# araray/sygnals

Hardware: AMD Instinct MI355X
Metric: Msamples/s STFT->MFCC (n_fft=2048, hop=512) (higher is better)
Workload: dtype f32; 1 GPU; C2: 1024 x 1 s @ 48 kHz clips per GPU, STFT n_fft=2048 hop=512 hann center -> 40-band Slaney mel -> power_to_db(ref=max, top_db=80) -> 13 MFCC (DCT-II ortho); clips_per_gpu=1024, clip_samples=48000, sr=48000, n_fft=2048, hop=512, n_mels=40, n_mfcc=13, rows_per_clip=13, parallelism=clip-sharded x1

## Files before the change

sygnals_amd/csrc/stft_mel.hip:

```cpp
#include "common.h"
#include <stdlib.h>
#include <string.h>

#define SETPRIO(n) __builtin_amdgcn_s_setprio(n)
#include "stft_dev.h"

namespace syg {
namespace {

constexpr bool X2_MEL = true;
constexpr int NFFT = 2048;
constexpr int MC = 1024;
constexpr int NBIN = 1025;
constexpr int MAXW = 16;
constexpr int P_STRIDE = 1090;
constexpr int PL2 = 132;
constexpr int SC_COMPLEX = 4 * PL2;
constexpr int TW2_STRIDE = 18;
constexpr int TW2_FLOATS = 4 * TW2_STRIDE * 2;
constexpr int TW1_FLOATS = 15 * 64 * 2;

struct MelPlan {
  int steps;
  int n_groups;
  int table_off;
};
constexpr int MTAB_INTS = 256;
constexpr int SEGTAB_WORDS = 2 * 2 * 64 * 4;
constexpr int SEGTAB4_WORDS = 2 * SEGTAB_WORDS;
constexpr int TRI4_ROW_BASE = 4;

struct ContrastPlan {
  int n_rows;
  int ascending;
  int lo[SYG_MAX_BANDS];
  int hi[SYG_MAX_BANDS];
  int k[SYG_MAX_BANDS];
};

typedef float v4f __attribute__((ext_vector_type(4)));

#include "row_features.h"

struct MfccArgs {
  const float* dct;
  const float* lifter;
  float* out;
  int n_mfcc;
  int ref_is_max;
  float ref_value, amin, top_db;
  int tp;
  int rows_per_clip;
};

__device__ __forceinline__ int x2g(int c, int cp) { return (cp & 7) * 16 + ((c + 4 * ((cp & 7) >> 1)) & 15); }

struct LaneConst {
  float2 twb[2];
  float2 cA2, cA3;
  int pkb[2];
  int pmb[2];
  int dA2, dA3;
  int kb[2];
  int g0[2], g1[2];
};

template <bool TWB = true>
__device__ __forceinline__ void init_lane_const(LaneConst& lc, int lane, const float2* __restrict__ twid) {
  constexpr float C1 = 0.92387953251128673848f, S1 = 0.38268343236508977173f, R = 0.70710678118654752440f;
#pragma unroll
  for (int j = 0; j < 2; ++j) {
    const int u = lane + 64 * j, c = u >> 3, cp = u & 7;
    int cm = 16 - c, cmp = 15 - cp;
    if (c == 0) { cm = 0; cmp = (cp == 0) ? 8 : 16 - cp; }
    lc.g0[j] = x2g(c, cp);
    lc.g1[j] = x2g(cm, cmp);
    const int kb = c + 16 * cp;
    lc.kb[j] = kb;
    lc.pkb[j] = ppos(kb);
    lc.pmb[j] = ppos(MC - kb);
    if (TWB) lc.twb[j] = twid[kb];
  }
  const bool sp = (lane == 0);
  lc.cA2 = sp ? make_float2(C1, -S1) : make_float2(0.f, -1.f);
  lc.cA3 = sp ? make_float2(S1, -C1) : make_float2(-R, -R);
  lc.dA2 = sp ? ppos(128) : 544;
  lc.dA3 = sp ? ppos(384) : 816;
}

template <int PD = 0, bool X2 = false>
__device__ __forceinline__ void wave_rfft2048(float2 (&v)[16], const LaneConst& lc, float2* __restrict__ sc,
                                             const float2* __restrict__ tw1l, const float2* __restrict__ tw2l,
                                             int lane, float2 (&xs)[2][4], float2 (&xm)[2][4], float2& x512 TARGS) {
  const int cl = lane >> 2, bp = lane & 3;
  dft16(v);
#pragma unroll
  for (int c = 1; c < 16; ++c) v[c] = cmul(v[c], tw1l[(c - 1) * 64 + lane]);
  TICK(1, v[1].x);
  float2 t[16];
  {
    const int r7 = cl & 7;
    const int rbase = r7 * 64 + bp + 8 * (cl & 8) / 2;
#pragma unroll
    for (int h = 0; h < 2; ++h) {
#pragma unroll
      for (int r = 0; r < 8; ++r) sc[r * 64 + (lane ^ (4 * r))] = v[8 * h + r];
      wave_lds_sync();
#pragma unroll
      for (int i = 0; i < 8; ++i) t[8 * h + i] = sc[rbase + 4 * (i ^ r7)];
      wave_lds_sync();
    }
#pragma unroll
    for (int i = 0; i < 8; ++i) {
      const auto sx = __builtin_amdgcn_permlane32_swap(__float_as_uint(t[i].x), __float_as_uint(t[8 + i].x), false, false);
      const auto sy = __builtin_amdgcn_permlane32_swap(__float_as_uint(t[i].y), __float_as_uint(t[8 + i].y), false, false);
      t[i] = make_float2(__uint_as_float(sx[0]), __uint_as_float(sy[0]));
      t[8 + i] = make_float2(__uint_as_float(sx[1]), __uint_as_float(sy[1]));
    }
  }
  TICK(2, t[0].x);
  SETPRIO(2 - PD > 0 ? 2 - PD : 0);
  dft16(t);
  {
    typedef __attribute__((address_space(3))) const v4f* lds_v4;
    lds_v4 t4 = (lds_v4)(tw2l + bp * TW2_STRIDE);
#pragma unroll
    for (int m = 0; m < 8; ++m) {
      const v4f tt = t4[m];
      if (m > 0) t[2 * m] = cmul(t[2 * m], make_float2(tt.x, tt.y));
      t[2 * m + 1] = cmul(t[2 * m + 1], make_float2(tt.z, tt.w));
    }
  }
  TICK(3, t[1].x);
  float2 G[2][4], H[2][4];
  {
    const int wbase = bp * PL2;
#pragma unroll
    for (int h = 0; h < 2; ++h) {
#pragma unroll
      for (int r = 0; r < 8; ++r) sc[wbase + r * 16 + ((cl + 4 * (r >> 1)) & 15)] = t[8 * h + r];
      wave_lds_sync();
#pragma unroll
      for (int j = 0; j < 2; ++j) {
        const float2* p = sc + (h == 0 ? lc.g0[j] : lc.g1[j]);
        if (h == 0) bfly4(p[0], p[PL2], p[2 * PL2], p[3 * PL2], G[j][0], G[j][1], G[j][2], G[j][3]);
        else bfly4(p[0], p[PL2], p[2 * PL2], p[3 * PL2], H[j][0], H[j][1], H[j][2], H[j][3]);
      }
      wave_lds_sync();
    }
  }
  TICK(4, G[0][0].x);
  SETPRIO(1 - PD > 0 ? 1 - PD : 0);
  x512 = X2 ? make_float2(2.f * G[0][2].x, -2.f * G[0][2].y)
            : make_float2(G[0][2].x, -G[0][2].y);
#pragma unroll
  for (int j = 0; j < 2; ++j) {
    float2 zk[4] = {G[j][0], G[j][1], G[j][2], G[j][3]};
    float2 zm[4] = {H[j][3], H[j][2], H[j][1], H[j][0]};
    if (j == 0) {
      const bool sp = (lane == 0);
      zk[2] = sp ? H[0][0] : zk[2];
      zk[3] = sp ? H[0][1] : zk[3];
      zm[0] = sp ? G[0][0] : zm[0];
      zm[1] = sp ? G[0][3] : zm[1];
      zm[2] = sp ? H[0][3] : zm[2];
      zm[3] = sp ? H[0][2] : zm[3];
    }
#pragma unroll
    for (int d = 0; d < 4; ++d) {
      const float2 E = make_float2(zk[d].x + zm[d].x, zk[d].y - zm[d].y);
      const float2 O = make_float2(zk[d].y + zm[d].y, zm[d].x - zk[d].x);
      constexpr float R = 0.70710678118654752440f;
      float2 rO;
      if (d == 0) rO = O;
      else if (d == 1) rO = make_float2(R * (O.x + O.y), R * (O.y - O.x));
      else if (j == 0) rO = cmul(O, d == 2 ? lc.cA2 : lc.cA3);
      else if (d == 2) rO = make_float2(O.y, -O.x);
      else rO = make_float2(R * (O.y - O.x), -R * (O.x + O.y));
      const float2 wO = cmul(lc.twb[j], rO);
      if (X2) {
        xs[j][d] = make_float2(E.x + wO.x, E.y + wO.y);
        xm[j][d] = make_float2(E.x - wO.x, wO.y - E.y);
      } else {
        xs[j][d] = make_float2(0.5f * (E.x + wO.x), 0.5f * (E.y + wO.y));
        xm[j][d] = make_float2(0.5f * (E.x - wO.x), -0.5f * (E.y - wO.y));
      }
    }
  }
}

template <int LOAD>
__device__ __forceinline__ void fetch_frame(float2 (&v)[16], const float* __restrict__ yb, int64_t L, int64_t s0,
                                            const float* __restrict__ stage_frame, int lane) {
  if (LOAD == 2) {
    const float2* sf = reinterpret_cast<const float2*>(stage_frame);
#pragma unroll
    for (int a = 0; a < 16; ++a) v[a] = sf[64 * a + lane];
    return;
  }
  const bool interior = (s0 >= 0) && (s0 + NFFT <= L);
  if (interior) {
#pragma unroll
    for (int a = 0; a < 16; ++a) {
      const int n = 64 * a + lane;
      if (LOAD == 1) v[a] = *reinterpret_cast<const float2*>(yb + s0 + 2 * n);
      else v[a] = make_float2(yb[s0 + 2 * n], yb[s0 + 2 * n + 1]);
    }
  } else {
#pragma unroll
    for (int a = 0; a < 16; ++a) {
      const int64_t s = s0 + 2 * (64 * a + lane);
      v[a].x = (s >= 0 && s < L) ? yb[s] : 0.f;
      v[a].y = (s + 1 >= 0 && s + 1 < L) ? yb[s + 1] : 0.f;
    }
  }
}

__device__ __forceinline__ void apply_window(float2 (&v)[16], const float2* __restrict__ winl, int lane) {
#pragma unroll
  for (int a = 0; a < 16; ++a) {
    const float2 wv = winl[64 * a + lane];
    v[a] = make_float2(v[a].x * wv.x, v[a].y * wv.y);
  }
}

template <int WAVES>
__device__ __forceinline__ void stage_tile(const float* yb, int clip_bytes, float* stage, int s_begin, int span,
                                           bool wide, int w, int lane) {
  typedef __attribute__((address_space(3))) void* lds_ptr;
  const auto rs = __builtin_amdgcn_make_buffer_rsrc(const_cast<float*>(yb), 0, clip_bytes, 0x00020000);
  if (wide) {
    const int n = (span + 255) >> 8;
    for (int c = w; c < n; c += WAVES)
      __builtin_amdgcn_raw_ptr_buffer_load_lds(rs, (lds_ptr)(stage + c * 256), 16, (s_begin + c * 256 + lane * 4) * 4,
                                               0, 0, 0);
  } else {
    const int n = (span + 63) >> 6;
    for (int c = w; c < n; c += WAVES)
      __builtin_amdgcn_raw_ptr_buffer_load_lds(rs, (lds_ptr)(stage + c * 64), 4, (s_begin + c * 64 + lane) * 4, 0, 0,
                                               0);
  }
}
__device__ __forceinline__ MfccArgs uni(const MfccArgs& a) {
  MfccArgs u;
  u.dct = uni(a.dct); u.lifter = uni(a.lifter); u.out = uni(a.out); u.n_mfcc = uni(a.n_mfcc);
  u.ref_is_max = uni(a.ref_is_max); u.ref_value = uni(a.ref_value); u.amin = uni(a.amin); u.top_db = uni(a.top_db);
  u.tp = uni(a.tp); u.rows_per_clip = uni(a.rows_per_clip);
  return u;
}

typedef __attribute__((address_space(3))) float* lds_fptr;
#include "mel_segments.h"

template <int WAVES>
__device__ __noinline__ void clip_dct(int clipmel_addr, int red_addr, int dct_addr, MfccArgs mfv, int n_mels_v, int T_v, int b_v,
                                      int w_v, int lane, int stride_v = WAVES) {
  const MfccArgs mf = uni(mfv);
  const int n_mels = uni(n_mels_v), T = uni(T_v), w = uni(w_v), stride = uni(stride_v);
  const int64_t b = uni(b_v);
  lds_fptr clipmel = (lds_fptr)(uintptr_t)(uint32_t)uni(clipmel_addr);
  lds_fptr red = (lds_fptr)(uintptr_t)(uint32_t)uni(red_addr);
  lds_fptr dctl = (lds_fptr)(uintptr_t)(uint32_t)uni(dct_addr);
  lds_fptr lifl = dctl + mf.n_mfcc * n_mels;
  float m = red[lane & (WAVES - 1)];
  m = fmaxf(m, dpp_f<DPP_QP_1032>(m));
  m = fmaxf(m, dpp_f<DPP_QP_2301>(m));
  m = fmaxf(m, dpp_f<DPP_ROW_HALF_MIRROR>(m));
  m = fmaxf(m, dpp_f<DPP_ROW_MIRROR>(m));
  constexpr float DB_PER_LOG2 = 3.01029995663981195f;
  const float ref = mf.ref_is_max ? m : fabsf(mf.ref_value);
  const float reflog = __builtin_amdgcn_logf(fmaxf(mf.amin, ref));
  const float flo = (mf.top_db >= 0.f) ? DB_PER_LOG2 * (__builtin_amdgcn_logf(fmaxf(mf.amin, m)) - reflog) - mf.top_db
                                       : -3.4e38f;
  const int ktiles = (mf.n_mfcc + 15) >> 4, ttiles = mf.tp >> 4;
  const int f = lane & 15, g = lane >> 4;
  for (int ot = w; ot < ktiles * ttiles; ot += stride) {
    const int kt = ot / ttiles, tq = ot - kt * ttiles;
    const int krow = kt * 16 + f, tcol = tq * 16 + f;
    v4f acc = {0.f, 0.f, 0.f, 0.f};
    for (int m0 = 0; m0 < n_mels; m0 += 16) {
      float a[4], bv[4];
#pragma unroll
      for (int i = 0; i < 4; ++i) {
        const int mm = m0 + 4 * i + g;
        const bool ok = mm < n_mels;
        a[i] = (krow < mf.n_mfcc && ok) ? dctl[krow * n_mels + mm] : 0.f;
        bv[i] = ok ? clipmel[mm * mf.tp + tcol] : 1.f;
      }
#pragma unroll
      for (int i = 0; i < 4; ++i) {
        const float db = fmaxf(DB_PER_LOG2 * (__builtin_amdgcn_logf(fmaxf(mf.amin, bv[i])) - reflog), flo);
        acc = __builtin_amdgcn_mfma_f32_16x16x4f32(a[i], db, acc, 0, 0, 0);
      }
    }
#pragma unroll
    for (int r = 0; r < 4; ++r) {
      const int k = kt * 16 + 4 * g + r;
      if (k < mf.n_mfcc && tcol < T) {
        float val = acc[r];
        if (mf.lifter) val *= lifl[k];
        mf.out[(b * mf.rows_per_clip + k) * (int64_t)T + tcol] = val;
      }
    }
  }
}

template <int WAVES, bool SLAB = true, int NPASS = 2>
struct Lds {
  static constexpr int TILE_T = WAVES;
  static constexpr int O_P = (NPASS == 4) ? 16 : 0;
  static constexpr int P_FLOATS = O_P + TILE_T * P_STRIDE + 16;
  static constexpr int SLAB_FLOATS = SLAB ? WAVES * 16 * TILE_T : 0;
  static constexpr int SEG_WORDS = NPASS * (SEGTAB_WORDS / 2);
  static constexpr int CPL_FLOATS = SLAB ? 3 * SYG_MAX_BANDS + MTAB_INTS : SEG_WORDS + 3 * SYG_MAX_BANDS;
  static constexpr int STAGE_FLOATS = (WAVES - 1) * 512 + NFFT;
  static constexpr int O_SLAB = P_FLOATS;
  static constexpr int O_TW2 = O_SLAB + SLAB_FLOATS;
  static constexpr int O_TW1 = O_TW2 + TW2_FLOATS;
  static constexpr int O_CPL = O_TW1 + TW1_FLOATS;
  static constexpr int O_WIN = O_CPL + CPL_FLOATS;
  static constexpr int O_STAGE = O_WIN + NFFT;
  static constexpr int TOTAL = O_STAGE + STAGE_FLOATS;
  static_assert(SC_COMPLEX * 2 <= P_STRIDE, "exchange scratch must fit inside a power row");
  static_assert(O_TW2 % 4 == 0 && O_WIN % 4 == 0 && O_STAGE % 4 == 0 && O_CPL % 4 == 0, "16-byte aligned LDS sections");
};

template <int WAVES, int LOAD, int MODE>
__global__ __launch_bounds__(WAVES * 64, 4) void stft2048_kernel(
    const float* __restrict__ y, int64_t L, int64_t ldy, int hop, int pad, int64_t T, int tiles_per_clip,
    int64_t total_tiles, int tiles_per_wg, const float2* __restrict__ win2, const float2* __restrict__ twid,
    const float* __restrict__ wpacked, MelPlan plan, int n_mels, float* __restrict__ mel_out, float binhz,
    float roll_percent, float bw_p, int smask, float* __restrict__ stats_out, ContrastPlan cplan,
    float* __restrict__ contrast_out, float2* __restrict__ cout, int dma_wide, MfccArgs mf) {
  constexpr bool TRIMEL = (MODE >= 8 && MODE <= 11);
  constexpr bool TRI = (MODE == 6 || MODE == 7 || TRIMEL);
  constexpr int NPASS = (MODE == 8 || MODE == 9) ? 4 : 2;
  constexpr int TRI_ROW_BASE = (NPASS == 4) ? TRI4_ROW_BASE : 0;
  typedef Lds<WAVES, !TRI, NPASS> LM;
  constexpr int SEG_WORDS = LM::SEG_WORDS;
  constexpr int NTHREADS = WAVES * 64;
  constexpr int TILE_T = WAVES;
  constexpr bool COMPLEX_OUT = (MODE == 2);
  constexpr bool ROWFN = (MODE == 1 || MODE == 7 || MODE == 9 || MODE == 11);
  constexpr bool CLIPM = (MODE == 3 || MODE == 6 || MODE == 7);
  constexpr bool X2 = X2_MEL && (MODE == 0 || MODE == 3 || MODE == 6 || MODE == 8 || MODE == 10);
#ifdef SYG_DEV_NO_RELC
  constexpr bool RELC = false;
#else
  constexpr bool RELC = (MODE == 7);
#endif
  constexpr float MELSC = X2 ? 0.25f : 1.f;
  extern __shared__ __attribute__((aligned(16))) float lds[];
  float* Pbuf = lds + LM::O_P;
  float* slab = lds + LM::O_SLAB;
  float2* tw2l = reinterpret_cast<float2*>(lds + LM::O_TW2);
  float2* tw1l = reinterpret_cast<float2*>(lds + LM::O_TW1);
  int* cpl = reinterpret_cast<int*>(lds + LM::O_CPL);
  int* cplc = TRI ? cpl + SEG_WORDS : cpl;
  float2* winl = reinterpret_cast<float2*>(lds + LM::O_WIN);
  float* stage = lds + LM::O_STAGE;
  float* clipmel = lds + (LOAD == 2 ? LM::TOTAL : LM::O_STAGE);
  float* tri_red = clipmel + 2 * n_mels * mf.tp;
  float* tri_dct = tri_red + 2 * WAVES;

  const int tid = threadIdx.x, lane = tid & 63;
  const int w = __builtin_amdgcn_readfirstlane(tid >> 6);

  const int64_t tile_begin = (int64_t)blockIdx.x * tiles_per_wg;
  const int64_t tile_end = (tile_begin + tiles_per_wg < total_tiles) ? tile_begin + tiles_per_wg : total_tiles;
  if (tile_begin >= tile_end) return;

  auto clip_of = [&](int64_t tile) { return (uint32_t)tile / (uint32_t)tiles_per_clip; };
  auto t0_of = [&](int64_t tile, uint32_t cq) {
    return (int64_t)((uint32_t)tile - cq * (uint32_t)tiles_per_clip) * TILE_T;
  };
  const int span = (TILE_T - 1) * hop + NFFT;
  auto dma = [&](int64_t tile) {
    const uint32_t cq = clip_of(tile);
    int ld = lane;
    asm volatile("" : "+v"(ld));
    stage_tile<WAVES>(y + (int64_t)cq * ldy, (int)(L * 4), stage, (int)(t0_of(tile, cq) * hop) - pad, span,
                      dma_wide != 0, w, ld);
  };
  if (LOAD == 2) dma(tile_begin);

  LaneConst lc;
  init_lane_const(lc, lane, twid);
  float* prow = Pbuf + w * P_STRIDE;
  float2* sc = reinterpret_cast<float2*>(prow);
  if (tid < 64) tw2l[(tid >> 4) * TW2_STRIDE + (tid & 15)] = twid[32 * (tid >> 4) * (tid & 15)];
  for (int i = tid; i < 15 * 64; i += NTHREADS) tw1l[i] = twid[2 * (i & 63) * ((i >> 6) + 1)];
  for (int i = tid; i < NFFT / 2; i += NTHREADS) winl[i] = win2[i];
  if (CLIPM) {
    if (TRI)
      for (int i = tid; i < 2 * n_mels * mf.tp; i += NTHREADS) clipmel[i] = 0.f;
    float* dctl = TRI ? tri_dct : clipmel + n_mels * mf.tp + WAVES;
    for (int i = tid; i < mf.n_mfcc * n_mels; i += NTHREADS) dctl[i] = mf.dct[i];
    if (mf.lifter != nullptr && tid < mf.n_mfcc) dctl[mf.n_mfcc * n_mels + tid] = mf.lifter[tid];
  }

  int* mtab = cpl + 3 * SYG_MAX_BANDS;
  if (!COMPLEX_OUT) {
    for (int i = tid; i < LM::P_FLOATS + LM::SLAB_FLOATS; i += NTHREADS) lds[i] = 0.f;
    if (TRI && wpacked != nullptr) {
      const int band_bytes = (TRIMEL ? (int)T : mf.tp) * 4;
      for (int i = tid; i < SEG_WORDS; i += NTHREADS) {
        int v = reinterpret_cast<const int*>(wpacked)[i];
        if ((i & 3) == 1 && ((i >> 8) & 1) == 0 && v >= 0) v *= band_bytes;
        cpl[i] = v;
      }
    }
    if (!TRI || ROWFN) {
#pragma unroll
      for (int r = 0; r < SYG_MAX_BANDS; ++r)
        if (tid == r) { cplc[r] = cplan.lo[r]; cplc[SYG_MAX_BANDS + r] = cplan.hi[r]; cplc[2 * SYG_MAX_BANDS + r] = cplan.k[r]; }
    }
    if (!TRI)
      for (int i = tid; i < MTAB_INTS; i += NTHREADS) mtab[i] = reinterpret_cast<const int*>(wpacked)[plan.table_off + i];
  }
  if (LOAD == 2) asm volatile("s_waitcnt vmcnt(0)" ::: "memory");
  __syncthreads();

  float cmax = 0.f;
  int64_t pend_b = -1;
  int cur = 0;
  bool tri_scan8 = false;
  if (TRI && wpacked != nullptr) {
    unsigned lk = 0;
#pragma unroll
    for (int p = 0; p < NPASS; ++p) lk |= (unsigned)(cpl[4 * (128 * p + lane) + 2] | cpl[4 * (128 * p + lane) + 3]);
    tri_scan8 = __builtin_amdgcn_ballot_w64((lk >> 24) != 0) != 0;
  }
  const int tri_ndct = ((mf.n_mfcc + 15) >> 4) * (mf.tp >> 4);
  const int tri_idle = (TRI && !TRIMEL) ? mf.tp - (int)T : 0;
  const bool tri_defer = TRI && !TRIMEL && tri_idle > 0 && (tri_ndct + tri_idle - 1) / (tri_idle > 0 ? tri_idle : 1) <= 3;
  float2 v[16];
  bool have = false;
  auto fetch = [&](int64_t tile) {
    const uint32_t cq = clip_of(tile);
    const int64_t t = t0_of(tile, cq) + w;
    have = t < T;
    int lf = lane;
    asm volatile("" : "+v"(lf));
    if (have) fetch_frame<LOAD>(v, y + (int64_t)cq * ldy, L, t * (int64_t)hop - pad, stage + w * hop, lf);
  };
  if (LOAD == 2) {
    fetch(tile_begin);
    __syncthreads();
    if (tile_begin + 1 < tile_end) dma(tile_begin + 1);
  }

#if SYG_DEV
  unsigned long long tacc[12] = {0, 0, 0, 0, 0, 0, 0, 0, 0, 0, 0, 0}, tprev;
  asm volatile("s_memtime %0\n\ts_waitcnt lgkmcnt(0)" : "=s"(tprev)::"memory");
#endif
#pragma unroll 1
  for (int64_t tile = tile_begin; tile < tile_end; ++tile) {
    const uint32_t cq = clip_of(tile);
    const int64_t b = cq;
    const int64_t t0 = t0_of(tile, cq);
    const int64_t t = t0 + w;
    if (LOAD != 2) fetch(tile);
    constexpr int PD = 1;
    SETPRIO(3 - PD);
    constexpr int NPRE = 7;
    const int ng = plan.steps >> 2;
    const float4* wp4w = reinterpret_cast<const float4*>(wpacked) + (int64_t)w * ng * 64;
    float4 apre[NPRE];
    if (have) {
      int lv = lane;
      asm volatile("" : "+v"(lv));
      if (RELC) init_lane_const<false>(lc, lv, twid);
      apply_window(v, winl, lv);
      TICK(0, v[0].x);
      float2 xs[2][4], xm[2][4], x512;
      wave_rfft2048<PD, X2>(v, lc, sc, tw1l, tw2l, lv, xs, xm, x512 TPASS);
      if (COMPLEX_OUT) {
        float2* o = cout + (b * T + t) * NBIN;
#pragma unroll
        for (int u = 0; u < 2; ++u)
#pragma unroll
          for (int d = 0; d < 4; ++d) {
            int k = lc.kb[u] + 256 * d;
            if (u == 0 && d >= 2 && lane == 0) k = (d == 2) ? 128 : 384;
            o[k] = xs[u][d];
            o[MC - k] = xm[u][d];
          }
        if (lane == 0) o[512] = x512;
      } else {
        int dA2 = lc.dA2, dA3 = lc.dA3;
        if (TRI && ROWFN) asm volatile("" : "+v"(dA2), "+v"(dA3));
#pragma unroll
        for (int u = 0; u < 2; ++u)
#pragma unroll
          for (int d = 0; d < 4; ++d) {
            const int off = (u == 0 && d == 2) ? dA2 : (u == 0 && d == 3) ? dA3 : 272 * d;
            prow[lc.pkb[u] + off] = fmaf(xs[u][d].x, xs[u][d].x, xs[u][d].y * xs[u][d].y);
            prow[lc.pmb[u] - off] = fmaf(xm[u][d].x, xm[u][d].x, xm[u][d].y * xm[u][d].y);
          }
        if (lane == 0) prow[ppos(512)] = fmaf(x512.x, x512.x, x512.y * x512.y);
      }
    } else if (!COMPLEX_OUT && !TRI) {
      for (int k = lane; k < P_STRIDE; k += 64) prow[k] = 0.f;
    }
    SETPRIO(0);
    if (COMPLEX_OUT) continue;
    if (TRI) {
      SETPRIO(3);
      const bool mine = (t < T);
      const bool clip_done = (t0 + TILE_T >= T);
      float* cmc = clipmel + cur * (n_mels * mf.tp);
      auto project = [&]() {
        int la = lane;
        asm volatile("" : "+v"(la)::"memory");
        wave_lds_sync();
        if (TRIMEL) {
          char* colg = reinterpret_cast<char*>(mel_out + (b * n_mels) * T + t);
          tri_project<NPASS>(prow - TRI_ROW_BASE, reinterpret_cast<const float4*>(cpl), la, tri_scan8,
                         [&](int boff, float v) { *reinterpret_cast<float*>(colg + boff) = MELSC * v; });
        } else {
          char* colb = reinterpret_cast<char*>(cmc + (int)t);
          tri_project<2>(prow, reinterpret_cast<const float4*>(cpl), la, tri_scan8, [&](int boff, float v) {
            *reinterpret_cast<float*>(colb + boff) = v;
            asm("v_max_f32_e32 %0, %0, %1" : "+v"(cmax) : "v"(v));
// ... 595 lines not shown
```

Before: 338,300 Msamples/s.

## Use ds_write_addtid for FFT LDS exchanges with permuted lane-to-column mapping

Replaces the per-lane scattered LDS writes in the two wave-level FFT transpose stages with inline-asm ds_write_addtid_b32 stores, which write lane-contiguous rows using M0-based addressing. Reads become paired float2 loads of split real/imag rows. To make this work, the lane-to-column mapping is permuted via p1col throughout the frame fetch, windowing and twiddle lookup, and the per-lane constants are reworked with a packed lookup. It aims to cut LDS instruction count and address arithmetic, at the cost of fragile inline asm, manual M0 handling and a more intricate index mapping.

```diff
diff --git a/sygnals_amd/csrc/stft_mel.hip b/sygnals_amd/csrc/stft_mel.hip
--- a/sygnals_amd/csrc/stft_mel.hip
+++ b/sygnals_amd/csrc/stft_mel.hip
@@ -14,8 +14,7 @@
 constexpr int NBIN = 1025;
 constexpr int MAXW = 16;
 constexpr int P_STRIDE = 1090;
-constexpr int PL2 = 132;
-constexpr int SC_COMPLEX = 4 * PL2;
+constexpr int SC_COMPLEX = 528;
 constexpr int TW2_STRIDE = 18;
 constexpr int TW2_FLOATS = 4 * TW2_STRIDE * 2;
 constexpr int TW1_FLOATS = 15 * 64 * 2;
@@ -53,7 +52,39 @@
   int rows_per_clip;
 };
 
-__device__ __forceinline__ int x2g(int c, int cp) { return (cp & 7) * 16 + ((c + 4 * ((cp & 7) >> 1)) & 15); }
+constexpr int X1_ROW = 130;
+constexpr int X2_ROW = 132;
+static_assert(7 * X1_ROW + 128 <= 2 * SC_COMPLEX && 7 * X2_ROW + 128 <= 2 * SC_COMPLEX, "exchange rows must fit the scratch");
+constexpr unsigned long long UNIT_C = 0xdb53ea62f971c840ull;
+__device__ __forceinline__ int p1col(int l) { return 4 * (l & 15) + ((l >> 4) ^ ((l >> 2) & 2)); }
+__device__ __forceinline__ int x2rho(int c7) { return ((c7 & 3) << 1) | (c7 >> 2); }
+__device__ __forceinline__ int x2g(int c, int cp) { return X2_ROW * (cp & 7) + 32 * (c >> 3) + 2 * x2rho(c & 7); }
+
+#pragma clang diagnostic push
+#pragma clang diagnostic ignored "-Winline-asm"
+template <int ROW>
+__device__ __forceinline__ void addtid_rows(uint32_t m0, const float2* x) {
+#define SYG_ADDTID(d, o) "ds_write_addtid_b32 %" #d " offset:%" #o "\n\t"
+  asm volatile("s_mov_b32 m0, %0\n\t"
+               "s_nop 0\n\t"
+               SYG_ADDTID(1, 17) SYG_ADDTID(2, 25)
+               SYG_ADDTID(3, 18) SYG_ADDTID(4, 26)
+               SYG_ADDTID(5, 19) SYG_ADDTID(6, 27)
+               SYG_ADDTID(7, 20) SYG_ADDTID(8, 28)
+               SYG_ADDTID(9, 21) SYG_ADDTID(10, 29)
+               SYG_ADDTID(11, 22) SYG_ADDTID(12, 30)
+               SYG_ADDTID(13, 23) SYG_ADDTID(14, 31)
+               SYG_ADDTID(15, 24) SYG_ADDTID(16, 32)
+               :: "s"(m0), "v"(x[0].x), "v"(x[0].y), "v"(x[1].x), "v"(x[1].y), "v"(x[2].x), "v"(x[2].y),
+                  "v"(x[3].x), "v"(x[3].y), "v"(x[4].x), "v"(x[4].y), "v"(x[5].x), "v"(x[5].y), "v"(x[6].x),
+                  "v"(x[6].y), "v"(x[7].x), "v"(x[7].y),
+                  "n"(0), "n"(4 * ROW), "n"(8 * ROW), "n"(12 * ROW), "n"(16 * ROW), "n"(20 * ROW), "n"(24 * ROW),
+                  "n"(28 * ROW), "n"(256), "n"(4 * ROW + 256), "n"(8 * ROW + 256), "n"(12 * ROW + 256),
+                  "n"(16 * ROW + 256), "n"(20 * ROW + 256), "n"(24 * ROW + 256), "n"(28 * ROW + 256)
+               : "memory", "m0");
+#undef SYG_ADDTID
+}
+#pragma clang diagnostic pop
 
 struct LaneConst {
   float2 twb[2];
@@ -70,7 +101,7 @@
   constexpr float C1 = 0.92387953251128673848f, S1 = 0.38268343236508977173f, R = 0.70710678118654752440f;
 #pragma unroll
   for (int j = 0; j < 2; ++j) {
-    const int u = lane + 64 * j, c = u >> 3, cp = u & 7;
+    const int c = (int)((uint32_t)(UNIT_C >> (32 * j)) >> (4 * (lane >> 3))) & 15, cp = lane & 7;
     int cm = 16 - c, cmp = 15 - cp;
     if (c == 0) { cm = 0; cmp = (cp == 0) ? 8 : 16 - cp; }
     lc.g0[j] = x2g(c, cp);
@@ -92,22 +123,31 @@
 __device__ __forceinline__ void wave_rfft2048(float2 (&v)[16], const LaneConst& lc, float2* __restrict__ sc,
                                              const float2* __restrict__ tw1l, const float2* __restrict__ tw2l,
                                              int lane, float2 (&xs)[2][4], float2 (&xm)[2][4], float2& x512 TARGS) {
-  const int cl = lane >> 2, bp = lane & 3;
+  const int col = p1col(lane);
+  const int hi = lane >> 5, rho = (lane >> 1) & 7, bp = ((lane >> 3) & 2) | (lane & 1);
+  const int c7 = (rho >> 1) | ((rho & 1) << 2);
+  const float* scf = reinterpret_cast<const float*>(sc);
+  typedef __attribute__((address_space(3))) const float* lds_cfptr;
+  const uint32_t m0 = __builtin_amdgcn_readfirstlane((uint32_t)(uintptr_t)(lds_cfptr)scf);
   dft16(v);
 #pragma unroll
-  for (int c = 1; c < 16; ++c) v[c] = cmul(v[c], tw1l[(c - 1) * 64 + lane]);
+  for (int c = 1; c < 16; ++c) v[c] = cmul(v[c], tw1l[(c - 1) * 64 + col]);
   TICK(1, v[1].x);
   float2 t[16];
   {
-    const int r7 = cl & 7;
-    const int rbase = r7 * 64 + bp + 8 * (cl & 8) / 2;
+    const float* rd = scf + X1_ROW * c7 + 8 * hi + 16 * (bp ^ (2 * hi));
 #pragma unroll
     for (int h = 0; h < 2; ++h) {
-#pragma unroll
-      for (int r = 0; r < 8; ++r) sc[r * 64 + (lane ^ (4 * r))] = v[8 * h + r];
+      addtid_rows<X1_ROW>(m0, v + 8 * h);
       wave_lds_sync();
 #pragma unroll
-      for (int i = 0; i < 8; ++i) t[8 * h + i] = sc[rbase + 4 * (i ^ r7)];
+      for (int i = 0; i < 4; ++i) {
+        if (i > 0) asm volatile("" ::: "memory");
+        const float2 re = *reinterpret_cast<const float2*>(rd + 2 * i);
+        const float2 im = *reinterpret_cast<const float2*>(rd + 64 + 2 * i);
+        t[8 * h + 2 * i] = make_float2(re.x, im.x);
+        t[8 * h + 2 * i + 1] = make_float2(re.y, im.y);
+      }
       wave_lds_sync();
     }
 #pragma unroll
@@ -134,17 +174,19 @@
   TICK(3, t[1].x);
   float2 G[2][4], H[2][4];
   {
-    const int wbase = bp * PL2;
 #pragma unroll
     for (int h = 0; h < 2; ++h) {
-#pragma unroll
-      for (int r = 0; r < 8; ++r) sc[wbase + r * 16 + ((cl + 4 * (r >> 1)) & 15)] = t[8 * h + r];
+      addtid_rows<X2_ROW>(m0, t + 8 * h);
       wave_lds_sync();
 #pragma unroll
       for (int j = 0; j < 2; ++j) {
-        const float2* p = sc + (h == 0 ? lc.g0[j] : lc.g1[j]);
-        if (h == 0) bfly4(p[0], p[PL2], p[2 * PL2], p[3 * PL2], G[j][0], G[j][1], G[j][2], G[j][3]);
-        else bfly4(p[0], p[PL2], p[2 * PL2], p[3 * PL2], H[j][0], H[j][1], H[j][2], H[j][3]);
+        const float* p = scf + (h == 0 ? lc.g0[j] : lc.g1[j]);
+        const float2 r01 = *reinterpret_cast<const float2*>(p), i01 = *reinterpret_cast<const float2*>(p + 64);
+        const float2 r23 = *reinterpret_cast<const float2*>(p + 16), i23 = *reinterpret_cast<const float2*>(p + 80);
+        const float2 z0 = make_float2(r01.x, i01.x), z1 = make_float2(r01.y, i01.y);
+        const float2 z2 = make_float2(r23.x, i23.x), z3 = make_float2(r23.y, i23.y);
+        if (h == 0) bfly4(z0, z1, z2, z3, G[j][0], G[j][1], G[j][2], G[j][3]);
+        else bfly4(z0, z1, z2, z3, H[j][0], H[j][1], H[j][2], H[j][3]);
       }
       wave_lds_sync();
     }
@@ -192,24 +234,25 @@
 template <int LOAD>
 __device__ __forceinline__ void fetch_frame(float2 (&v)[16], const float* __restrict__ yb, int64_t L, int64_t s0,
                                             const float* __restrict__ stage_frame, int lane) {
+  const int col = p1col(lane);
   if (LOAD == 2) {
     const float2* sf = reinterpret_cast<const float2*>(stage_frame);
 #pragma unroll
-    for (int a = 0; a < 16; ++a) v[a] = sf[64 * a + lane];
+    for (int a = 0; a < 16; ++a) v[a] = sf[64 * a + col];
     return;
   }
   const bool interior = (s0 >= 0) && (s0 + NFFT <= L);
   if (interior) {
 #pragma unroll
     for (int a = 0; a < 16; ++a) {
-      const int n = 64 * a + lane;
+      const int n = 64 * a + col;
       if (LOAD == 1) v[a] = *reinterpret_cast<const float2*>(yb + s0 + 2 * n);
       else v[a] = make_float2(yb[s0 + 2 * n], yb[s0 + 2 * n + 1]);
     }
   } else {
 #pragma unroll
     for (int a = 0; a < 16; ++a) {
-      const int64_t s = s0 + 2 * (64 * a + lane);
+      const int64_t s = s0 + 2 * (64 * a + col);
       v[a].x = (s >= 0 && s < L) ? yb[s] : 0.f;
       v[a].y = (s + 1 >= 0 && s + 1 < L) ? yb[s + 1] : 0.f;
     }
@@ -217,9 +260,10 @@
 }
 
 __device__ __forceinline__ void apply_window(float2 (&v)[16], const float2* __restrict__ winl, int lane) {
+  const int col = p1col(lane);
 #pragma unroll
   for (int a = 0; a < 16; ++a) {
-    const float2 wv = winl[64 * a + lane];
+    const float2 wv = winl[64 * a + col];
     v[a] = make_float2(v[a].x * wv.x, v[a].y * wv.y);
   }
 }
```

New measurement: 352,400 Msamples/s (median of 6 runs). 4.2% higher.
